# Pyrokine/LineSegmentDetector-SLAM

Measured on AMD Instinct MI355X. Metric: Mpixels/sec LSD (grad+grow+NFA), higher is better.
Workload: dtype f64; 1 GPU; 512 x 2048x2048 u8 occupancy maps per GPU tiled/rolled/flipped from 4 aisle-class fixtures (SURVEY 8d C4), full pipeline incl. lineIm, params 0.3/0.6/22.5/0.7/1024; images_total=512, images_rank0=512, parallelism=single GPU, rccl_gather_in_step=False, steps_in_flight=8, steps_in_flight_asked=8, region_waves_per_image=4, help_across_workgroups=False, last_steps_with_help=0, writeback_map=False

## Files before the change

### include/lsd_hip.h

```cpp
#ifndef LSD_HIP_H
#define LSD_HIP_H
#include <stddef.h>
#include <stdint.h>

#ifdef __cplusplus
extern "C" {
#endif

#define LSD_ABI_VERSION 1

enum {
    LSD_OK = 0,
    LSD_ERR_INVALID = 1,
    LSD_ERR_NO_DEVICE = 2,
    LSD_ERR_HIP = 3,
    LSD_ERR_UNSUPPORTED = 4,
    LSD_ERR_CAPACITY = 5,
    LSD_ERR_NOMEM = 6,
    LSD_ERR_INTERNAL = 7
};

typedef struct lsd_params {
    double sca;
    double sig;
// ... 236 lines not shown
                      const lsd_grid_match_rec *records, lsd_map_param map_param, double range_max, const uint8_t *corr,
                      double ang_step, lsd_grid_response_par response, lsd_grid_response_rec *out, uint32_t *volume);

void lsd_scaled_size(int cols, int rows, double sca, int *w, int *h);

enum { LSD_STAGE_ALL = 0, LSD_STAGE_GAUSS = 1, LSD_STAGE_GRAD = 2, LSD_STAGE_SORT = 3, LSD_STAGE_REGION = 4 };
int lsd_set_stop_after(lsd_ctx *ctx, int stage);
int lsd_set_trace(lsd_ctx *ctx, int on);
int lsd_set_fused_front(lsd_ctx *ctx, int on);
int lsd_set_region_waves(lsd_ctx *ctx, int waves);
int lsd_set_region_help(lsd_ctx *ctx, int waves);
int lsd_set_cost_history(lsd_ctx *ctx, int on);
int lsd_debug_set_stamp_budget(lsd_ctx *ctx, unsigned grows);
int lsd_debug_set_tuning(lsd_ctx *ctx, const char *name, int value);

enum { LSD_DBG_GAUSS = 1, LSD_DBG_MAG, LSD_DBG_DEG, LSD_DBG_STATE, LSD_DBG_ORDER, LSD_DBG_ORDER_VAL,
       LSD_DBG_NB, LSD_DBG_MAXGRAD, LSD_DBG_RECS, LSD_DBG_SEEDS, LSD_DBG_NSEED, LSD_DBG_STATS };
int lsd_debug_fetch(lsd_ctx *ctx, int image, int what, void *out, size_t bytes);

int lsd_debug_eval_math(lsd_ctx *ctx, int fn, const double *a, const double *b, double *out0, double *out1, size_t n);

int lsd_debug_lines(lsd_ctx *ctx, const double *recs, int n, int cols, int rows, lsd_line *lines_out, uint8_t *line_im);

int lsd_debug_calibrate(lsd_ctx *ctx, size_t bytes);

int lsd_last_timings(lsd_ctx *ctx, float ms_out[6]);

#ifdef __cplusplus
}
#endif
#endif
```

### linesegmentdetector-slam_amd/__init__.py

```python
import ctypes as C
import os

import numpy as np

_HERE = os.path.dirname(os.path.abspath(__file__))
LIB_PATH = os.path.join(_HERE, "liblsdhip.so")

LSD_OK, LSD_ERR_INVALID, LSD_ERR_NO_DEVICE, LSD_ERR_HIP, LSD_ERR_UNSUPPORTED, LSD_ERR_CAPACITY, LSD_ERR_NOMEM, LSD_ERR_INTERNAL = range(8)
LSD_FLAG_WRITEBACK_MAP = 1
STAGE_ALL, STAGE_GAUSS, STAGE_GRAD, STAGE_SORT, STAGE_REGION = range(5)
(DBG_GAUSS, DBG_MAG, DBG_DEG, DBG_STATE, DBG_ORDER, DBG_ORDER_VAL, DBG_NB, DBG_MAXGRAD, DBG_RECS, DBG_SEEDS,
 DBG_NSEED, DBG_STATS) = range(1, 13)

lsd_sca, lsd_sig, lsd_angThre, lsd_denThre, pseBin = 0.3, 0.6, 22.5, 0.7, 1024
z_occ_max_dis = 1.0
HOST_MAX_LINES_DEFAULT = 8192
rdp_leastPoint, rdp_threLine, rdp_leastDist = 3, 0.08, 0.5


class lsd_params(C.Structure):
    _fields_ = [("sca", C.c_double), ("sig", C.c_double), ("angThre", C.c_double), ("denThre", C.c_double),
                ("pseBin", C.c_int)]


# ... 162 lines not shown
    "lsd_enqueue_fa_carry_rebase_device": (_i, [_vp, _vp, _i, _vp, C.c_int32, lsd_map_frame, lsd_map_frame, _vp]),
    "lsd_enqueue_map_update_device": (_i, [_vp, _vp, _i, _i, _dbl, _dbl, _ppar, _vp, _vp, _vp, _i, _vp, _vp, _vp]),
    "lsd_reserve_map_update": (_i, [_vp, _i, _i]),
    "lsd_enqueue_scan_ingest_device": (_i, [_vp, _vp, _i, _i, _vp, _vp, _vp, _i, _vp]),
    "lsd_enqueue_laserscan_ingest_device": (_i, [_vp, _vp, _vp, _i, _i, _vp, _vp, _vp, _i, _vp]),
    "lsd_enqueue_grid_integrate_device": (_i, [_vp, _vp, _vp, _i, _i, _vp, _sz, lsd_map_param, _dbl, _vp, _vp, _vp]),
    "lsd_enqueue_grid_publish_device": (_i, [_vp, _vp, _vp, _sz, C.c_uint32, C.c_uint32, C.c_uint32, _vp, _vp]),
    "lsd_grid_integrate": (_i, [_vp, _vp, _vp, _i, _i, _vp, lsd_map_param, _dbl, _vp, _vp]),
    "lsd_enqueue_grid_likelihood_device": (_i, [_vp, _vp, _vp, _i, _i, C.c_uint32, C.c_uint32, C.c_uint32, lsd_grid_smear, _vp, _vp]),
    "lsd_grid_smear_default": (_i, [_dbl, _i, C.POINTER(lsd_grid_smear)]),
    "lsd_enqueue_grid_match_device": (_i, [_vp, _vp, _vp, _i, _i, _vp, _sz, lsd_map_param, _dbl, _vp, lsd_grid_search, _vp, _vp]),
    "lsd_grid_match": (_i, [_vp, _vp, _vp, _i, _i, _vp, lsd_map_param, _dbl, _vp, lsd_grid_search, _vp]),
    "lsd_grid_coarse_bytes": (_sz, [_i, _i, _i]),
    "lsd_enqueue_grid_coarse_device": (_i, [_vp, _vp, _i, _i, _i, _vp, _vp]),
    "lsd_enqueue_grid_match_mr_device": (_i, [_vp, _vp, _vp, _i, _i, _vp, _sz, lsd_map_param, _dbl, _vp, _vp, _i, lsd_grid_search, _vp, _vp, _vp]),
    "lsd_grid_match_mr": (_i, [_vp, _vp, _vp, _i, _i, _vp, lsd_map_param, _dbl, _vp, _i, lsd_grid_search, _vp, _vp]),
    "lsd_grid_response_volume_bytes": (_sz, [_i, lsd_grid_response]),
    "lsd_enqueue_grid_response_device": (_i, [_vp, _vp, _vp, _i, _i, _vp, _sz, _vp, lsd_map_param, _dbl, _vp, _dbl, lsd_grid_response, _vp, _vp,
                                              _vp]),
    "lsd_grid_response": (_i, [_vp, _vp, _vp, _i, _i, _vp, _vp, lsd_map_param, _dbl, _vp, _dbl, lsd_grid_response, _vp, _vp]),
    "lsd_debug_calibrate": (_i, [_vp, _sz]),
    "lsd_debug_eval_math": (_i, [_vp, _i, _vp, _vp, _vp, _vp, _sz]),
    "lsd_debug_lines": (_i, [_vp, _vp, _i, _i, _i, _vp, _vp]),
}
EXPORTED_SYMBOLS = list(_ABI)
del _vp, _i, _sz, _dbl, _pi, _ppar, _localize_args, _live_map_args, _maps_args

_lib = None


def load_library(path=None):
    global _lib
    if _lib is not None and path is None:
        return _lib
    p = path or os.environ.get("LSD_HIP_LIB") or LIB_PATH
    try:
        import torch
    except ImportError:
        pass
    if not os.path.exists(p):
        raise ImportError("liblsdhip.so is not built (%s); run `python -c 'import __graft_entry__ as g; g.build()'` "
                          "-- there is no CPU fallback" % p)
    L = C.CDLL(p)
    for name, (restype, argtypes) in _ABI.items():
        try:
            fn = getattr(L, name)
# ... 489 lines not shown
        if what == DBG_STATE:
            return get(what, np.uint32, npx).reshape(h, w)
        if what == DBG_NB:
            return int(get(what, np.int32, 1)[0])
        if what == DBG_NSEED:
            return int(get(what, np.int32, 1)[0])
        if what == DBG_MAXGRAD:
            return float(get(what, np.float64, 1)[0])
        if what == DBG_ORDER:
            return get(what, np.uint32, npx)[:self.fetch(image, DBG_NB, shape_wh)]
        if what == DBG_ORDER_VAL:
            return get(what, np.uint16, npx)[:self.fetch(image, DBG_NB, shape_wh)]
        if what == DBG_STATS:
            v = get(what, np.int64, 48)
            d = dict(zip(("grow_calls", "grown_px", "nfa_calls", "rrr_calls", "rrr_passes", "rrr_sentinel_drops",
                          "rrr_oob_reads", "cycles_refill", "cycles_total", "cycles_grow", "cycles_rect",
                          "cycles_nfa", "cycles_mark", "small_bails", "wait_noslot", "seeds", "exact_angle_evals",
                          "tile_fetches", "batches", "cycles_tiles", "spec_redos", "spec_discards", "cycles_wait", "small_steps",
                          "refill_rounds", "cycles_eval", "cycles_sums", "cycles_refine", "cycles_small", "cycles_select", "cycles_commit",
                          "wait_noseed", "requeued_ahead", "cycles_eval_at_cursor", "depth_end", "nfa_min_abs_enc", "nfa_min_gap_enc", "help_exports", "help_evals", "near_ties",
                          "wd_commit", "wd_next", "wd_nseeds", "wd_state", "wd_nbig", "wd_lock", "wd_pend", "wd_wave"),
                         [int(x) for x in v]))
            d["set_answers"], d["sets_founded"] = int(v[41]), int(v[42])
            d["cycles_nfa_count"], d["nfa_tail_iters"] = int(v[43]), int(v[44])
            d["nfa_bracket_misses"] = int(v[40])
            for k in ("nfa_min_abs", "nfa_min_gap"):
                enc = d.pop(k + "_enc")
                d[k] = float("inf") if enc == 0 else float(np.array([0x7ff0000000000000 - enc], np.uint64).view(np.float64)[0])
            return d
        if what == DBG_SEEDS:
            ns = self.fetch(image, DBG_NSEED, shape_wh)
            return get(what, SEED_DTYPE, ns)
        raise ValueError(what)

    def eval_math(self, fn, a, b=None):
        a = np.ascontiguousarray(a, np.float64)
        b = None if b is None else np.ascontiguousarray(b, np.float64)
        o0, o1 = np.zeros_like(a), np.zeros_like(a)
        self._chk(self.L.lsd_debug_eval_math(self.h, fn, a.ctypes.data, None if b is None else b.ctypes.data,
                                             o0.ctypes.data, o1.ctypes.data, a.size))
        return o0, o1

    def debug_lines(self, recs, rows, cols, want_lineim=True):
        r = np.ascontiguousarray(recs, np.float64).reshape(-1, 4)
        lines = np.zeros(len(r), LINE_DTYPE)
        im = np.zeros((rows, cols), np.uint8) if want_lineim else None
        self._chk(self.L.lsd_debug_lines(self.h, r.ctypes.data, len(r), cols, rows, lines.ctypes.data, im.ctypes.data if want_lineim else None))
        return lines, im

    def fetch_recs(self, image, count):
        a = np.zeros(max(count * 12, 1), np.float64)
        self._chk(self.L.lsd_debug_fetch(self.h, image, DBG_RECS, a.ctypes.data, a.nbytes))
        return a[:count * 12].reshape(count, 12)


class structLSD:

    def __init__(self, lineIm, linesInfo):
        self.lineIm = lineIm
        self.linesInfo = linesInfo
        self.len_linesInfo = len(linesInfo)


_default_ctx = None


def default_context():
    global _default_ctx
    if _default_ctx is None:
        _default_ctx = Context(0)
    return _default_ctx
# ... 1063 lines not shown
```

### linesegmentdetector-slam_amd/csrc/k_region.hip

```cpp
#include "lsd_internal.h"
#include "devmath.h"

#ifndef LSD_REGION_NW
#define LSD_REGION_NW 4
#endif
#if LSD_REGION_NW == 8
#define RVAR w8
#else
#define RVAR w4
#endif

namespace lsdhip {
namespace RVAR {
#include "region/config.h"
#include "region/stats.h"
#include "region/lds.h"
#include "region/wave.h"
#include "region/tiles.h"
#include "region/grow.h"
#include "region/rect.h"
#include "region/nfa.h"
#include "region/eval.h"

#ifdef LSD_REGION_STATS
// ... 921 lines not shown
            P[22] = (double)((long long)(precise ? n1 + 1 : 0) + 32768ll * n2 + 32768ll * 32768ll * m_off);
            P[23] = (double)epoch_snap;
            rg.aux[k & (RW - 1)] = (uint32_t)(wave * NS + slot);
        }
        wg_fence();
        if (lane == 0) st_st(&rg.state[k & (RW - 1)], R_STASH);
        adv = true;
    }

    asm volatile("s_waitcnt vmcnt(0)" ::: "memory");
    if (wave == 0 && lane == 0 && !pool) {
        b.counts[img] = lds_ld(&s_abort) ? -1 : s_lines;
        if (b.nseed) b.nseed[img] = s_ntrace;
    }
    if (b.stats && !pool) {
        unsigned long long* st = reinterpret_cast<unsigned long long*>(b.stats + img * kStatWords);
        if (lane == 0 && wave == 0 && !lds_ld(&s_abort)) { b.stats[img * kStatWords + 45] = (long long)(__builtin_amdgcn_s_getreg((3 << 11) | 20) & 15); b.stats[img * kStatWords + 46] = rt_begin; b.stats[img * kStatWords + 47] = (long long)__builtin_amdgcn_s_memrealtime(); }
        if (lane == 0 && wave == 0) {
            long long tot = (long long)__builtin_amdgcn_s_memtime() - t_begin;
            const long long rt = ((long long)__builtin_amdgcn_s_memrealtime() - rt_begin) * 24;
            if (tot <= 0 || tot > 4 * rt + 1000000) tot = rt > 0 ? rt : 1;
            g_stat[c.wave][sslot(ST_TOTAL)] = (unsigned long long)tot; g_stat[c.wave][sslot(ST_SEEDS)] = (unsigned long long)nseeds; DSTAT(ST_DEPTHEND, lds_ld(&s_depth));
        }
        if (lane < ST_COUNT && !lds_ld(&s_abort) && (sslot(lane) != 11 || lane == ST_NFASLOW || kStatSlots == ST_COUNT)) {
            if (lane == ST_MINNFA || lane == ST_MINGAP) atomicMax(&st[lane], g_stat[c.wave][sslot(lane)]);
            else atomicAdd(&st[lane], g_stat[c.wave][sslot(lane)]);
        }
        g_stat[c.wave][sslot(ST_XHELP)] = 0ull;
        g_stat[c.wave][sslot(ST_MINNFA)] = 0ull; g_stat[c.wave][sslot(ST_MINGAP)] = 0ull; g_stat[c.wave][sslot(ST_NFASLOW)] = 0ull; g_stat[c.wave][sslot(ST_TIES)] = 0ull;
    }
    if (!b.xq) return;
    if (wave == 0 && !pool) {
        agent_release();
        if (lane == 0) { st_l2(&xr[2], 1u); atomicAdd(&xhdr[1], 1u); }
    }
    bool early = !pool && ld_l2(&xhdr[0]) < (uint32_t)nimg;
    if (early) {
        if (b.tun_early <= 0) return;
        int ok = 0;
        if (lane == 0) {
            if (atomicAdd(&xhdr[3], 1u) >= (uint32_t)(b.tun_early * NW)) atomicSub(&xhdr[3], 1u);
            else ok = 1;
        }
        if (!__builtin_amdgcn_readfirstlane(ok)) return;
    }

    if (lane < NS) slot_k_l = -1;
    int hx = -1, hj = 0, hidle = 0, hscan = 0;
// ... 136 lines not shown
#undef LT

__global__ __launch_bounds__(64 * NW, LSD_REGION_WAVES_PER_SIMD) void k_region(Geom g, Buffers b, uint32_t id_base) {
#if LSD_REGION_NW == 8
    __shared__ int s_take;
    while (true) {
        int bid = (int)blockIdx.x, nimg = (int)gridDim.x - b.npool;
        if (b.pcount) {
            if (threadIdx.x == 0) s_take = atomicAdd(b.pcount, 1);
            __syncthreads();
            bid = s_take; nimg = b.nimg;
            __syncthreads();
            if (bid >= nimg) return;
        }
        region_image(g, b, id_base, bid, nimg);
        if (!b.pcount) return;
        __syncthreads();
    }
#else
    region_image(g, b, id_base, (int)blockIdx.x, (int)gridDim.x - b.npool);
#endif
}

}

#if LSD_REGION_NW == 8
void launch_region_w8(const Geom& g, const Buffers& b, int n, uint32_t id_base, hipStream_t s) {
    hipLaunchKernelGGL(w8::k_region, dim3(n + b.npool), dim3(64 * w8::NW), 0, s, g, b, id_base);
}
int region_slots() { return w8::NS; }
int region_waves() { return w8::NW; }
int region_ring() { return w8::RW; }
#else
void launch_region_w4(const Geom& g, const Buffers& b, int n, uint32_t id_base, hipStream_t s) {
    hipLaunchKernelGGL(w4::k_region, dim3(n + b.npool), dim3(64 * w4::NW), 0, s, g, b, id_base);
}
#endif

}
```

### linesegmentdetector-slam_amd/csrc/lsd_ctx.hip

```cpp
#include <math.h>
#include <stddef.h>
#include <stdio.h>
#include <stdlib.h>
#include <string.h>

#include <algorithm>
#include <mutex>
#include <string>
#include <vector>

#include "lsd_devbuf.h"
#include "lsd_internal.h"
#include "k1_lds.h"
#include "k_rdp_lds.h"

using namespace lsdhip;

struct Workspace {
    size_t cap_gpx = 0;
    size_t cap_n = 0, cap_npx = 0, cap_ws = 0;
    int cap_max_lines = 0;
    DevBuf<double> gauss, mag, deg, recs, recs_scaled;
    DevBuf<double2> sc;
    DevBuf<uint32_t> order;
// ... 1746 lines not shown
    HIPCHK(c, hipMemcpy(out0, d0.get(), n * 8, hipMemcpyDeviceToHost));
    HIPCHK(c, hipMemcpy(out1, d1.get(), n * 8, hipMemcpyDeviceToHost));
    return LSD_OK;
}

int lsd_debug_lines(lsd_ctx* c, const double* recs, int n, int cols, int rows, lsd_line* lines_out, uint8_t* line_im) {
    if (!c || !recs || !lines_out || n <= 0 || cols <= 0 || rows <= 0) return LSD_ERR_INVALID;
    HIPCHK(c, hipSetDevice(c->device));
    DevBuf<double> dr; DevBuf<int32_t> dn; DevBuf<lsd_line> dl; DevBuf<uint8_t> di;
    const size_t px = (size_t)cols * rows;
    HIPCHK(c, dr.resize((size_t)n * 4)); HIPCHK(c, dn.resize(1)); HIPCHK(c, dl.resize(n));
    if (line_im) HIPCHK(c, di.resize(px));
    HIPCHK(c, hipMemcpy(dr.get(), recs, (size_t)n * 4 * 8, hipMemcpyHostToDevice));
    HIPCHK(c, hipMemcpy(dn.get(), &n, 4, hipMemcpyHostToDevice));
    HIPCHK(c, hipMemsetAsync(dl.get(), 0xFF, (size_t)n * sizeof(lsd_line), c->stream));
    if (line_im) launch_clear(di.get(), px, c->num_cus, c->stream);
    launch_lines_of(dr.get(), dn.get(), dl.get(), line_im ? di.get() : nullptr, n, cols, rows, c->stream);
    HIPCHK(c, hipStreamSynchronize(c->stream));
    HIPCHK(c, hipMemcpy(lines_out, dl.get(), (size_t)n * sizeof(lsd_line), hipMemcpyDeviceToHost));
    if (line_im) HIPCHK(c, hipMemcpy(line_im, di.get(), px, hipMemcpyDeviceToHost));
    return LSD_OK;
}

}
```

### linesegmentdetector-slam_amd/csrc/lsd_internal.h

```cpp
#pragma once
#include <hip/hip_runtime.h>
#include <stdint.h>
#include "../../include/lsd_hip.h"

namespace lsdhip {

constexpr double kPi = 3.14159265358979323846;
constexpr int kCentreCount = 32768;
constexpr int kMaxTapRadius = 40;
constexpr int kLgTable = 16384;
constexpr int kLgTableMax = 1 << 23;
constexpr int kStatWords = 48;
constexpr int kStatTiesWord = 39;
constexpr int kStatTotalWord = 8;
constexpr int kPTable = 16;
constexpr int kXStride = 768, kXReq = 64, kXHdr = 16;

struct Geom {
    int W, H;
    int w, h;
    int npx;
    int gp;
    double sca;
    int tapR;
// ... 65 lines not shown
    int lg_count;
    const double* ptab;
    void* seeds;
    int32_t* nseed;
    long long* stats;
};

struct SeedRec {
    int order_idx, x, y, num, outcome, final_num;
    double logNFA;
};

hipError_t prepare_gauss(const Geom& g);
void launch_gauss(const Geom& g, const Buffers& b, int n, uint8_t* clr, bool remapped, hipStream_t s);
bool front_fits(const Geom& g, size_t max_lds);
void launch_front(const Geom& g, const Buffers& b, int n, uint8_t* clr, hipStream_t s);
void launch_remap_writeback(const Geom& g, const Buffers& b, int n, hipStream_t s);
void launch_gradient(const Geom& g, const Buffers& b, int n, hipStream_t s);
void launch_sort(const Geom& g, const Buffers& b, int n, hipStream_t s);
void launch_ordv(const double* mag, const unsigned long long* maxbits, const uint32_t* ord, uint16_t* out, int count, int pseBin, hipStream_t s);
void launch_order(const Buffers& b, int n, int npx, const long long* hist, hipStream_t s);
void launch_region_w4(const Geom& g, const Buffers& b, int n, uint32_t id_base, hipStream_t s);
void launch_region_w8(const Geom& g, const Buffers& b, int n, uint32_t id_base, hipStream_t s);
int region_slots();
int region_waves();
int region_ring();
void launch_calib(double* buf, size_t n, hipStream_t s);
void launch_match(const double* map_cache, int cols, int rows, const lsd_line* map_lines, const lsd_line* scan_lines,
                  const double* pts, int n_points, double lidx, double lidy, double lastx, double lasty, const int* pairs,
                  int n_pairs, double zmax, double max_esti_dist, double* out, hipStream_t s);
void launch_occ_to_map(const uint8_t* in, uint8_t* out, size_t n, hipStream_t s);
void launch_mapcache_spread(const uint8_t* maps, double* out, unsigned long long* claim, uint32_t* fr_a, uint32_t* fr_b, int* ctl,
                            int* cnt, int n, int G, int W, int H, double res, double zmax, int cell_radius, hipStream_t s);
void launch_mapcache(const uint8_t* maps, double* out, unsigned long long* claim, uint32_t* fr_a, uint32_t* fr_b, int n,
                     int W, int H, double res, double zmax, int cell_radius, hipStream_t s);
void launch_lines(const Geom& g, const Buffers& b, int n, hipStream_t s);
void launch_lines_of(const double* recs_scaled, const int32_t* count, lsd_line* lines, uint8_t* line_im, int n, int W, int H, hipStream_t s);
void launch_clear(uint8_t* p, size_t bytes, int num_cus, hipStream_t s);
void launch_compact_lines(const lsd_line* lines, const int32_t* counts, int max_lines, int n, lsd_line* flat, int32_t* offsets, hipStream_t s);
void launch_rdp(const double* scans, const int* lens, int n, int stride, int oriMapCol, int oriMapRow, double mapResol, double mapOriX,
                double mapOriY, int region_point_limit, double thre_line, double line_dist_thre_m, lsd_line* lines_out, int* n_lines,
                double* pts_out, int pts_cap, int* n_pts, double* lidar_pos, int* im_size, hipStream_t s);
void launch_rdp_maps(const double* scans, const int* lens, int n, int stride, const lsd_map_ref* maps, int n_maps, const int32_t* map_of,
                     int scans_per_seq, int region_point_limit, double thre_line, double line_dist_thre_m, lsd_line* lines_out, int* n_lines,
                     double* pts_out, int pts_cap, int* n_pts, double* lidar_pos, int* im_size, hipStream_t s);
int rdp_max_len();
// ... 62 lines not shown
```

### linesegmentdetector-slam_amd/csrc/region/nfa.h

```cpp
__device__ __forceinline__ double log_gamma_dev(const double* lgamma, int lg_count, int x) {
    if (x >= 0 && x < lg_count) return lgamma[x];
    const double xd = x;
    return 0.918938533204673 + (xd - 0.5) * log(xd) - xd +
           0.5 * xd * log(xd * sinh(1.0 / xd) + 1.0 / (810 * pow(xd, 6.0)));
}

template <int NP>
__device__ __forceinline__ int nfa_count(const RCtx& c, const Rec& rec, const double (&prec)[NP], int (&ali)[NP]) {
    const int lane = c.lane, xLim = c.w, yLim = c.h;
    STAT(ST_NFA, NP);
    [[maybe_unused]] const long long t00 = NOW();
    double verX[4], verY[4];
    verX[0] = rec.x1 - rec.dy * rec.wid / 2.0;
    verX[1] = rec.x2 - rec.dy * rec.wid / 2.0;
    verX[2] = rec.x2 + rec.dy * rec.wid / 2.0;
    verX[3] = rec.x1 + rec.dy * rec.wid / 2.0;
    verY[0] = rec.y1 + rec.dx * rec.wid / 2.0;
    verY[1] = rec.y2 + rec.dx * rec.wid / 2.0;
    verY[2] = rec.y2 - rec.dx * rec.wid / 2.0;
    verY[3] = rec.y1 - rec.dx * rec.wid / 2.0;
    int offset;
    if ((rec.x1 < rec.x2) && (rec.y1 <= rec.y2)) offset = 0;
    else if ((rec.x1 >= rec.x2) && (rec.y1 < rec.y2)) offset = 1;
    else if ((rec.x1 > rec.x2) && (rec.y1 >= rec.y2)) offset = 2;
    else offset = 3;
    const double vx0 = verX[offset & 3], vx1 = verX[(offset + 1) & 3], vx2 = verX[(offset + 2) & 3],
                 vx3 = verX[(offset + 3) & 3];
    const double vy0 = verY[offset & 3], vy1 = verY[(offset + 1) & 3], vy2 = verY[(offset + 2) & 3],
                 vy3 = verY[(offset + 3) & 3];
    const double cx0 = ceil(vx0);
    int xlen = cvt_x86(cx0 - floor(vx2));
    if (xlen < 0 && xlen != (int)0x80000000) xlen = -xlen;
    xlen = (int)((unsigned)xlen + 1u);
    const double k0 = (vy1 - vy0) / (vx1 - vx0);
    const double k1 = (vy2 - vy1) / (vx2 - vx1);
    const double k2 = (vy2 - vy3) / (vx2 - vx3);
    const double k3 = (vy3 - vy0) / (vx3 - vx0);
    int all = 0;
    #pragma unroll
    for (int q = 0; q < NP; q++) ali[q] = 0;
    const bool axis0 = axis_exact(rec.dx, rec.dy);
    const double ex_ = rec.x2 - rec.x1, ey_ = rec.y2 - rec.y1;
    const double cnz = kTieCoord * (fabs(rec.x1) + fabs(rec.y1) + fabs(ex_) + fabs(ey_) + rec.wid + 1.0);
    int ties_a = 0;
    int ties = (lane == 0 && !axis0 && (fabs(vx0 - rint(vx0)) <= cnz || fabs(vx2 - rint(vx2)) <= cnz)) ? 1 : 0;
    int* const s_incl = reinterpret_cast<int*>(G_WL(c.wave));
    int* const s_lo = s_incl + 64;
    int* const s_x = s_incl + 128;
    for (int cb = 0; cb < xlen; cb += 64) {
        const int i = cb + lane;
        int cntc = 0, lo = 0, xr = 0;
        if (i < xlen) {
            xr = cvt_x86(i + cx0);
            int yLow, yHigh;
            const double eLow = xr < vx3 ? vy0 + (xr - vx0) * k3 : vy3 + (xr - vx3) * k2;
            const double eHigh = xr < vx1 ? vy0 + (xr - vx0) * k0 : vy1 + (xr - vx1) * k1;
            yLow = cvt_x86(ceil(eLow));
            yHigh = cvt_x86(floor(eHigh));
            const double kLow = xr < vx3 ? k3 : k2, kHigh = xr < vx1 ? k0 : k1;
            if (!axis0 && (fabs(eLow - rint(eLow)) <= cnz * (1.0 + fabs(kLow)) || fabs(eHigh - rint(eHigh)) <= cnz * (1.0 + fabs(kHigh)) ||
                           fabs(xr - vx3) <= cnz || fabs(xr - vx1) <= cnz)) {
                ties++;
#ifdef LSD_TIE_PRINT
                printf("edge tie: xr %d eLow %.17g eHigh %.17g vx0 %.17g vx1 %.17g vx3 %.17g dx %.17g dy %.17g wid %.17g x1 %.17g y1 %.17g\n", xr, eLow, eHigh, vx0, vx1, vx3, rec.dx, rec.dy, rec.wid, rec.x1, rec.y1);
#endif
            }
            if (xr >= 0 && xr < xLim) {
                lo = yLow < 0 ? 0 : yLow;
                const int hi = yHigh > yLim - 1 ? yLim - 1 : yHigh;
                if (hi >= lo) cntc = hi - lo + 1;
            }
        }
        int inc = cntc;
        for (int off = 1; off < 64; off <<= 1) {
            const int t = __shfl_up(inc, off);
            if (lane >= off) inc += t;
        }
        const int tot = __builtin_amdgcn_readlane(inc, 63);
        if (tot == 0) continue;
        s_incl[lane] = inc; s_lo[lane] = lo; s_x[lane] = xr;
        all += tot;
        for (int t0 = 0; t0 < tot; t0 += 64) {
            const int t = t0 + lane;
            double df = 1e300;
            if (t < tot) {
                int ci = 0;
                for (int step = 32; step >= 1; step >>= 1)
                    if (s_incl[ci + step - 1] <= t) ci += step;
                const int ex = ci ? s_incl[ci - 1] : 0;
                const int j = s_lo[ci] + (t - ex);
                df = angle_diff(rec.deg, c.deg[(size_t)j * xLim + s_x[ci]]);
            }
            bool near = false;
            #pragma unroll
            for (int q = 0; q < NP; q++) {
                ali[q] += __builtin_popcountll(ballot64(df < prec[q]));
                near = near || fabs(df - prec[q]) <= 4.0 * kTieAng;
            }
            if (near) ties_a++;
        }
    }
    for (int off = 32; off >= 1; off >>= 1) { ties += __shfl_xor(ties, off); ties_a += __shfl_xor(ties_a, off); }
    TIES_AT(TS_EDGE, ties);
    TIES_AT(TS_ALIGN, ties_a);
    PSTAT(ST_NFACNT, NOW() - t00);
    return all;
}

struct NfaVal { double v; int flags; };
__device__ __noinline__ NfaVal nfa_tail(int all, int ali, int pk, double p, double logNT, const double* ptab, const double* lgamma, int lg_count) {
    if (all == 0 || ali == 0) return NfaVal{-logNT, 1};
    const double logp = ptab[pk * 3 + 0], log10p = ptab[pk * 3 + 1], log1mp = ptab[pk * 3 + 2];
    if (all == ali) return NfaVal{-logNT - all * log10p, 1};
    const double proTerm = p / (1.0 - p);
    const double log1Coef = log_gamma_dev(lgamma, lg_count, all + 1) - log_gamma_dev(lgamma, lg_count, ali + 1) - log_gamma_dev(lgamma, lg_count, all - ali + 1);
    const double log1Term = log1Coef + ali * logp + (all - ali) * log1mp;
    double term = exp_g(log1Term);
    const double eps = 2.2204e-16;
    if (fabs(term) < 100 * eps) {
        if (ali > all * p) return NfaVal{-log10_g(term) - logNT, 0};
        return NfaVal{-logNT, 1};
    }
    int nslow = 0;
    double binTail = term;
    const double tole = 0.1;
    constexpr double kOcmlBracket = 0x1p-44, kTiny = 0x1p-1000;
    for (int i = ali + 1; i <= all; i++) {
        const double binTerm = (all - i + 1) / (i * 1.0);
        const double multTerm = binTerm * proTerm;
        term *= multTerm;
        binTail += term;
        if (binTerm < 1) {
            const double N = (double)(all - i + 1), om = 1.0 - multTerm;
            const double Pd = pow(multTerm, N), Ld = log10(binTail);
            const double Pe = Pd * kOcmlBracket + kTiny, Le = fabs(Ld) * kOcmlBracket + kTiny;
            const double err_hi = term * ((1 - (Pd - Pe)) / om - 1), err_lo = term * ((1 - (Pd + Pe)) / om - 1);
            const double a1 = -(Ld - Le) - logNT, a2 = -(Ld + Le) - logNT;
            const double f1 = fabs(a1), f2 = fabs(a2);
            const double rhs_hi = tole * fmax(f1, f2) * binTail;
            const double rhs_lo = (a1 > 0) == (a2 > 0) && a1 != 0 && a2 != 0 ? tole * fmin(f1, f2) * binTail : 0.0;
            bool stop;
            if (err_hi < rhs_lo) stop = true;
            else if (!(err_lo < rhs_hi)) stop = false;
            else {
                nslow++;
                const double err = term * ((1 - pow_g(multTerm, N)) / om - 1);
                stop = err < tole * fabs(-log10_g(binTail) - logNT) * binTail;
            }
            if (stop) break;
        }
    }
    return NfaVal{-log10_g(binTail) - logNT, nslow << 8};
}

__device__ __noinline__ double improve(int cw_) {
    RCtx c = g_ctx[__builtin_amdgcn_readfirstlane(cw_)];
    c.lane = (int)(threadIdx.x & 63u);
    const int lane = c.lane;
    const double delt = 0.5, delt2 = delt / 2.0;
    Rec& best = g_ws[c.wave].rec;
    double bestNFA = 0;
    [[maybe_unused]] const long long t0 = NOW();
    auto margins = [&](double v, bool host_only, bool first) {
        if (fabs(v) <= 1.7976931348623157e308) {
            const double nv = 0x1p-51 * fabs(v + c.logNT) + 0x1p-52 * (1.0 + fmax(fabs(v), c.logNT));
            if (!host_only) STATMAX(ST_MINNFA, kInfBits - (unsigned long long)__double_as_longlong(fabs(v) / nv));
            int tie = (!host_only && fabs(v) / nv < 2.0) ? 1 : 0;
            if (!first && v != bestNFA) {
                const double nb = 0x1p-51 * fabs(bestNFA + c.logNT) + 0x1p-52 * (1.0 + fmax(fabs(bestNFA), c.logNT));
                STATMAX(ST_MINGAP, kInfBits - (unsigned long long)__double_as_longlong(fabs(v - bestNFA) / (nv + nb)));
                if (fabs(v - bestNFA) / (nv + nb) < 2.0) tie++;
            }
            TIES_AT(TS_NFA, tie);
        }
    };
    {
        Rec r = best;
        const double pr[1] = {r.prec};
        int al[1];
        const int all = nfa_count<1>(c, r, pr, al);
        const NfaVal nv = nfa_tail(all, al[0], r.pk, r.p, c.logNT, c.ptab, c.lgamma, c.lg_count);
        STAT(ST_NFASLOW, nv.flags >> 8);
        margins(nv.v, (nv.flags & 1) != 0, true);
        bestNFA = nv.v;
    }
    auto next_try = [&](Rec& r, int ph) -> bool {
        if (ph == 0 || ph == 4) { r.p /= 2.0; r.prec = r.p * kPi; r.pk++; return true; }
        if (!(r.wid - delt >= 0.5)) return false;
        if (ph == 2) { r.x1 -= r.dy * delt2; r.y1 += r.dx * delt2; r.x2 -= r.dy * delt2; r.y2 += r.dx * delt2; }
        else if (ph == 3) { r.x1 += r.dy * delt2; r.y1 -= r.dx * delt2; r.x2 += r.dy * delt2; r.y2 -= r.dx * delt2; }
        r.wid -= delt;
        return true;
    };
    for (int ph = 0; ph < 5 && !(bestNFA > 0); ph++) {
        int my_all = 0, my_ali = 0, my_pk = 0;
        double my_p = 0.0;
        bool my_eval = false;
        Rec r = best;
        if (ph == 0 || ph == 4) {
            double pr[5];
            int al[5];
            #pragma unroll
            for (int t = 0; t < 5; t++) pr[t] = r.p / (double)(2 << t) * kPi;
            const int all = nfa_count<5>(c, r, pr, al);
            #pragma unroll
            for (int t = 0; t < 5; t++)
                if (lane == t) { my_all = all; my_ali = al[t]; my_pk = r.pk + t + 1; my_p = r.p / (double)(2 << t); my_eval = true; }
        } else {
            for (int t = 0; t < 5; t++) {
                if (!next_try(r, ph)) continue;
                const double pr[1] = {r.prec};
                int al[1];
                const int all = nfa_count<1>(c, r, pr, al);
                if (lane == t) { my_all = all; my_ali = al[0]; my_pk = r.pk; my_p = r.p; my_eval = true; }
            }
        }
        NfaVal nv{0.0, 0};
        if (my_eval) nv = nfa_tail(my_all, my_ali, my_pk, my_p, c.logNT, c.ptab, c.lgamma, c.lg_count);
        r = best;
        for (int t = 0; t < 5; t++) {
            if (!next_try(r, ph)) continue;
            const double v = rl(nv.v, t);
            const int fl = __builtin_amdgcn_readlane(nv.flags, t);
            STAT(ST_NFASLOW, fl >> 8);
            margins(v, (fl & 1) != 0, false);
            if (v > bestNFA) { bestNFA = v; best = r; }
        }
    }
    PSTAT(ST_TNFA, NOW() - t0);
    return bestNFA;
}
```

### linesegmentdetector-slam_amd/csrc/region/stats.h

```cpp
enum { ST_GROW = 0, ST_GROWN, ST_NFA, ST_RRR, ST_RRRPASS, ST_SENT, ST_OOB, ST_TREFILL, ST_TOTAL, ST_TGROW, ST_TRECT, ST_TNFA,
       ST_TMARK, ST_SMALLBAIL, ST_WNOSLOT, ST_SEEDS, ST_EXACT, ST_WRING, ST_BATCHES, ST_TTILES, ST_REDO, ST_DISCARD,
       ST_WAIT, ST_SMALLSTEPS, ST_SLOW, ST_TEVAL, ST_TSUMS, ST_TREFINE, ST_TSMALL, ST_TSELECT, ST_TCOMMIT, ST_WNOSEED,
       ST_DEPTHUP, ST_DEPTHDN, ST_DEPTHEND, ST_MINNFA, ST_MINGAP, ST_XEXP, ST_XHELP, ST_TIES, ST_NFASLOW, ST_SETHIT, ST_SETNEW, ST_NFACNT, ST_NFAITER, ST_COUNT };
static_assert(ST_TOTAL == kStatTotalWord, "lsd_last_region_cycles reads this word");
static_assert(ST_TIES == kStatTiesWord, "lsd_last_sensitivity reads this word");
#ifdef LSD_REGION_STATS
constexpr int kStatSlots = ST_COUNT;
__device__ constexpr int sslot(int i) { return i; }
#else
constexpr int kStatSlots = 19;
__device__ constexpr int sslot(int i) {
    return i == ST_GROW ? 0 : i == ST_GROWN ? 1 : i == ST_NFA ? 2 : i == ST_RRR ? 3 : i == ST_RRRPASS ? 4 : i == ST_SENT ? 5 : i == ST_OOB ? 6 :
           i == ST_TOTAL ? 7 : i == ST_SEEDS ? 8 : i == ST_REDO ? 9 : i == ST_DISCARD ? 10 : i == ST_MINNFA ? 12 : i == ST_MINGAP ? 13 : i == ST_XEXP ? 14 : i == ST_XHELP ? 15 : i == ST_SETHIT ? 16 : i == ST_SETNEW ? 17 : i == ST_TIES ? 18 : 11;
}
#endif
#define STAT(i, v) do { g_stat[c.wave][sslot(i)] += (unsigned long long)(v); } while (0)
#define STATMAX(i, v) do { const unsigned long long n_ = (v); if (n_ > g_stat[c.wave][sslot(i)]) g_stat[c.wave][sslot(i)] = n_; } while (0)
constexpr unsigned long long kInfBits = 0x7ff0000000000000ull;
constexpr double kTieAng = 1e-15, kTieFlip = 1e-13, kTieRel = 1e-12, kTieCoord = 4e-15;
#ifdef LSD_TIE_SITES
__device__ constexpr unsigned long long tie_weight(int site) { unsigned long long w = 1; for (int i = 0; i < site; i++) w *= 1000ull; return w; }
#define TIE_UNIT(site) tie_weight(site)
#else
#define TIE_UNIT(site) 1ull
#endif
#define TIES_AT(site, v) STAT(ST_TIES, (unsigned long long)(v) * TIE_UNIT(site))
enum { TS_GROW = 0, TS_FLIP, TS_DENS, TS_DIST, TS_EDGE, TS_ALIGN, TS_NFA };
__device__ __forceinline__ bool axis_exact(double dx, double dy) { return fmin(fabs(dx), fabs(dy)) < 1e-15; }
#ifdef LSD_REGION_STATS
#define DSTAT(i, v) STAT(i, v)
#define NOW() ((long long)__builtin_amdgcn_s_memtime())
#else
#define DSTAT(i, v) do { } while (0)
#define NOW() 0ll
#endif
#ifdef LSD_REGION_BATCHPROF
#define BSTAT(i, v) DSTAT(i, v)
#define PSTAT(i, v) do { } while (0)
#else
#define BSTAT(i, v) do { } while (0)
#define PSTAT(i, v) DSTAT(i, v)
#endif
```

Baseline: 69120 Mpix/s.

## Count NFA pixels for all width/shift tries in one shared column sweep

For the width-reduction and shift phases of rectangle improvement, the change computes the pixel counts for all up to five candidate rectangles in one pass over the union of their columns. It records each try's row range in LDS and reads each gradient angle only once, instead of rescanning the image for every try. This is meant to cut repeated global loads and per-try scan overhead in improve(). In exchange it adds per-column recomputation of every try's rectangle geometry and a five-way membership test per pixel. It also adds a debug kernel that checks the counts and extra tail-timing stats, which only apply in stats builds.

New measurement: 68700 Mpix/s. No clear change (-0.6%).

```diff
diff --git a/include/lsd_hip.h b/include/lsd_hip.h
--- a/include/lsd_hip.h
+++ b/include/lsd_hip.h
@@ -282,6 +282,8 @@
 
 int lsd_debug_lines(lsd_ctx *ctx, const double *recs, int n, int cols, int rows, lsd_line *lines_out, uint8_t *line_im);
 
+int lsd_debug_nfa_counts(lsd_ctx *ctx, const double *deg, int cols, int rows, const double *recs, int n, int phase, int32_t *out);
+
 int lsd_debug_calibrate(lsd_ctx *ctx, size_t bytes);
 
 int lsd_last_timings(lsd_ctx *ctx, float ms_out[6]);
diff --git a/linesegmentdetector-slam_amd/__init__.py b/linesegmentdetector-slam_amd/__init__.py
--- a/linesegmentdetector-slam_amd/__init__.py
+++ b/linesegmentdetector-slam_amd/__init__.py
@@ -208,6 +208,7 @@
     "lsd_debug_calibrate": (_i, [_vp, _sz]),
     "lsd_debug_eval_math": (_i, [_vp, _i, _vp, _vp, _vp, _vp, _sz]),
     "lsd_debug_lines": (_i, [_vp, _vp, _i, _i, _i, _vp, _vp]),
+    "lsd_debug_nfa_counts": (_i, [_vp, _vp, _i, _i, _vp, _i, _i, _vp]),
 }
 EXPORTED_SYMBOLS = list(_ABI)
 del _vp, _i, _sz, _dbl, _pi, _ppar, _localize_args, _live_map_args, _maps_args
@@ -743,7 +744,8 @@
                           "wd_commit", "wd_next", "wd_nseeds", "wd_state", "wd_nbig", "wd_lock", "wd_pend", "wd_wave"),
                          [int(x) for x in v]))
             d["set_answers"], d["sets_founded"] = int(v[41]), int(v[42])
-            d["cycles_nfa_count"], d["nfa_tail_iters"] = int(v[43]), int(v[44])
+            d["cycles_nfa_count"] = int(v[43])
+            d["cycles_tail_exp"], d["cycles_tail_stop"], d["cycles_tail_log"] = (((int(v[44]) >> sh) & 0x1fffff) << 8 for sh in (0, 21, 42))
             d["nfa_bracket_misses"] = int(v[40])
             for k in ("nfa_min_abs", "nfa_min_gap"):
                 enc = d.pop(k + "_enc")
@@ -768,6 +770,15 @@
         im = np.zeros((rows, cols), np.uint8) if want_lineim else None
         self._chk(self.L.lsd_debug_lines(self.h, r.ctypes.data, len(r), cols, rows, lines.ctypes.data, im.ctypes.data if want_lineim else None))
         return lines, im
+
+    def debug_nfa_counts(self, deg, recs, phase):
+        if not hasattr(self.L, "lsd_debug_nfa_counts"):
+            raise LsdError(LSD_ERR_INVALID, "this liblsdhip.so predates lsd_debug_nfa_counts")
+        d = np.ascontiguousarray(deg, np.float64)
+        r = np.ascontiguousarray(recs, np.float64).reshape(-1, 12)
+        out = np.zeros((len(r), 2, 5, 2), np.int32)
+        self._chk(self.L.lsd_debug_nfa_counts(self.h, d.ctypes.data, d.shape[1], d.shape[0], r.ctypes.data, len(r), int(phase), out.ctypes.data))
+        return out
 
     def fetch_recs(self, image, count):
         a = np.zeros(max(count * 12, 1), np.float64)
diff --git a/linesegmentdetector-slam_amd/csrc/k_region.hip b/linesegmentdetector-slam_amd/csrc/k_region.hip
--- a/linesegmentdetector-slam_amd/csrc/k_region.hip
+++ b/linesegmentdetector-slam_amd/csrc/k_region.hip
@@ -967,8 +967,11 @@
             if (tot <= 0 || tot > 4 * rt + 1000000) tot = rt > 0 ? rt : 1;
             g_stat[c.wave][sslot(ST_TOTAL)] = (unsigned long long)tot; g_stat[c.wave][sslot(ST_SEEDS)] = (unsigned long long)nseeds; DSTAT(ST_DEPTHEND, lds_ld(&s_depth));
         }
-        if (lane < ST_COUNT && !lds_ld(&s_abort) && (sslot(lane) != 11 || lane == ST_NFASLOW || kStatSlots == ST_COUNT)) {
+        if (lane < ST_COUNT && !lds_ld(&s_abort) && (sslot(lane) != 11 || lane == ST_NFASLOW || kStatSlots >= ST_COUNT)) {
             if (lane == ST_MINNFA || lane == ST_MINGAP) atomicMax(&st[lane], g_stat[c.wave][sslot(lane)]);
+#ifdef LSD_REGION_STATS
+            else if (lane == ST_TAILPARTS) atomicAdd(&st[lane], tail_parts(g_stat[c.wave][ST_TTAILEXP], g_stat[c.wave][ST_TTAILSTOP], g_stat[c.wave][ST_TTAILLOG]));
+#endif
             else atomicAdd(&st[lane], g_stat[c.wave][sslot(lane)]);
         }
         g_stat[c.wave][sslot(ST_XHELP)] = 0ull;
@@ -1151,6 +1154,38 @@
 #endif
 }
 
+#if LSD_REGION_NW == 4
+__global__ __launch_bounds__(64) void k_nfa_counts(const double* deg, int w, int h, const double* recs, int n, int ph, int* out) {
+    RCtx c;
+    c.w = w; c.h = h; c.lane = (int)threadIdx.x; c.wave = 0; c.deg = deg;
+    const int lane = c.lane;
+    if (lane < kStatSlots) g_stat[0][lane] = 0ull;
+    for (int k = 0; k < n; k++) {
+        const double* f = recs + (size_t)k * 12;
+        Rec best;
+        best.x1 = f[0]; best.y1 = f[1]; best.x2 = f[2]; best.y2 = f[3]; best.wid = f[4]; best.cX = f[5]; best.cY = f[6]; best.deg = f[7];
+        best.dx = f[8]; best.dy = f[9]; best.p = f[10]; best.prec = f[11]; best.pk = 0;
+        int* const o = out + (size_t)k * 20;
+        Rec r = best;
+        int nt = 0;
+        for (int t = 0; t < 5; t++)
+            if (next_try(r, ph)) nt++;
+        int a = -1, b = -1;
+        if (nt >= 1 && !nfa_count_tries(c, best, ph, nt, a, b)) { a = -2; b = -2; }
+        if (lane < 5) { o[lane * 2] = lane < nt ? a : -1; o[lane * 2 + 1] = lane < nt ? b : -1; }
+        r = best;
+        for (int t = 0; t < 5; t++) {
+            int all = -1, al[1] = {-1};
+            if (next_try(r, ph)) {
+                const double pr[1] = {r.prec};
+                all = nfa_count<1>(c, r, pr, al);
+            }
+            if (lane == 0) { o[10 + t * 2] = all; o[10 + t * 2 + 1] = al[0]; }
+        }
+    }
+}
+#endif
+
 }
 
 #if LSD_REGION_NW == 8
@@ -1164,6 +1199,9 @@
 void launch_region_w4(const Geom& g, const Buffers& b, int n, uint32_t id_base, hipStream_t s) {
     hipLaunchKernelGGL(w4::k_region, dim3(n + b.npool), dim3(64 * w4::NW), 0, s, g, b, id_base);
 }
+void launch_nfa_counts(const double* deg, int w, int h, const double* recs, int n, int ph, int* out, hipStream_t s) {
+    hipLaunchKernelGGL(w4::k_nfa_counts, dim3(1), dim3(64), 0, s, deg, w, h, recs, n, ph, out);
+}
 #endif
 
 }
diff --git a/linesegmentdetector-slam_amd/csrc/lsd_ctx.hip b/linesegmentdetector-slam_amd/csrc/lsd_ctx.hip
--- a/linesegmentdetector-slam_amd/csrc/lsd_ctx.hip
+++ b/linesegmentdetector-slam_amd/csrc/lsd_ctx.hip
@@ -1792,4 +1792,23 @@
     return LSD_OK;
 }
 
-}
+int lsd_debug_nfa_counts(lsd_ctx* c, const double* deg, int cols, int rows, const double* recs, int n, int phase, int32_t* out) {
+    if (!c || !deg || !recs || !out || n <= 0 || cols <= 0 || rows <= 0 || cols >= 32766 || rows >= 32766 || phase < 1 || phase > 3) return LSD_ERR_INVALID;
+    for (int k = 0; k < n; k++) {
+        const double* f = recs + (size_t)k * 12;
+        for (int j = 0; j < 12; j++)
+            if (!(fabs(f[j]) <= (j == 8 || j == 9 ? 1.0000001 : 65536.0))) return LSD_ERR_INVALID;
+    }
+    HIPCHK(c, hipSetDevice(c->device));
+    DevBuf<double> dd, dr; DevBuf<int32_t> dout;
+    const size_t px = (size_t)cols * rows;
+    HIPCHK(c, dd.resize(px)); HIPCHK(c, dr.resize((size_t)n * 12)); HIPCHK(c, dout.resize((size_t)n * 20));
+    HIPCHK(c, hipMemcpy(dd.get(), deg, px * 8, hipMemcpyHostToDevice));
+    HIPCHK(c, hipMemcpy(dr.get(), recs, (size_t)n * 12 * 8, hipMemcpyHostToDevice));
+    launch_nfa_counts(dd.get(), cols, rows, dr.get(), n, phase, dout.get(), c->stream);
+    HIPCHK(c, hipStreamSynchronize(c->stream));
+    HIPCHK(c, hipMemcpy(out, dout.get(), (size_t)n * 20 * 4, hipMemcpyDeviceToHost));
+    return LSD_OK;
+}
+
+}
diff --git a/linesegmentdetector-slam_amd/csrc/lsd_internal.h b/linesegmentdetector-slam_amd/csrc/lsd_internal.h
--- a/linesegmentdetector-slam_amd/csrc/lsd_internal.h
+++ b/linesegmentdetector-slam_amd/csrc/lsd_internal.h
@@ -111,6 +111,7 @@
 void launch_order(const Buffers& b, int n, int npx, const long long* hist, hipStream_t s);
 void launch_region_w4(const Geom& g, const Buffers& b, int n, uint32_t id_base, hipStream_t s);
 void launch_region_w8(const Geom& g, const Buffers& b, int n, uint32_t id_base, hipStream_t s);
+void launch_nfa_counts(const double* deg, int w, int h, const double* recs, int n, int ph, int* out, hipStream_t s);
 int region_slots();
 int region_waves();
 int region_ring();
diff --git a/linesegmentdetector-slam_amd/csrc/region/nfa.h b/linesegmentdetector-slam_amd/csrc/region/nfa.h
--- a/linesegmentdetector-slam_amd/csrc/region/nfa.h
+++ b/linesegmentdetector-slam_amd/csrc/region/nfa.h
@@ -5,11 +5,13 @@
            0.5 * xd * log(xd * sinh(1.0 / xd) + 1.0 / (810 * pow(xd, 6.0)));
 }
 
-template <int NP>
-__device__ __forceinline__ int nfa_count(const RCtx& c, const Rec& rec, const double (&prec)[NP], int (&ali)[NP]) {
-    const int lane = c.lane, xLim = c.w, yLim = c.h;
-    STAT(ST_NFA, NP);
-    [[maybe_unused]] const long long t00 = NOW();
+struct RectScan {
+    double vx0, vx1, vx2, vx3, vy0, vy1, vy2, vy3, k0, k1, k2, k3, cx0, cnz;
+    int xlen;
+    bool axis0;
+};
+__device__ __forceinline__ RectScan rect_scan(const Rec& rec) {
+    RectScan s;
     double verX[4], verY[4];
     verX[0] = rec.x1 - rec.dy * rec.wid / 2.0;
     verX[1] = rec.x2 - rec.dy * rec.wid / 2.0;
@@ -24,26 +26,59 @@
     else if ((rec.x1 >= rec.x2) && (rec.y1 < rec.y2)) offset = 1;
     else if ((rec.x1 > rec.x2) && (rec.y1 >= rec.y2)) offset = 2;
     else offset = 3;
-    const double vx0 = verX[offset & 3], vx1 = verX[(offset + 1) & 3], vx2 = verX[(offset + 2) & 3],
-                 vx3 = verX[(offset + 3) & 3];
-    const double vy0 = verY[offset & 3], vy1 = verY[(offset + 1) & 3], vy2 = verY[(offset + 2) & 3],
-                 vy3 = verY[(offset + 3) & 3];
-    const double cx0 = ceil(vx0);
-    int xlen = cvt_x86(cx0 - floor(vx2));
+    s.vx0 = verX[offset & 3]; s.vx1 = verX[(offset + 1) & 3]; s.vx2 = verX[(offset + 2) & 3]; s.vx3 = verX[(offset + 3) & 3];
+    s.vy0 = verY[offset & 3]; s.vy1 = verY[(offset + 1) & 3]; s.vy2 = verY[(offset + 2) & 3]; s.vy3 = verY[(offset + 3) & 3];
+    s.cx0 = ceil(s.vx0);
+    int xlen = cvt_x86(s.cx0 - floor(s.vx2));
     if (xlen < 0 && xlen != (int)0x80000000) xlen = -xlen;
-    xlen = (int)((unsigned)xlen + 1u);
-    const double k0 = (vy1 - vy0) / (vx1 - vx0);
-    const double k1 = (vy2 - vy1) / (vx2 - vx1);
-    const double k2 = (vy2 - vy3) / (vx2 - vx3);
-    const double k3 = (vy3 - vy0) / (vx3 - vx0);
+    s.xlen = (int)((unsigned)xlen + 1u);
+    s.k0 = (s.vy1 - s.vy0) / (s.vx1 - s.vx0);
+    s.k1 = (s.vy2 - s.vy1) / (s.vx2 - s.vx1);
+    s.k2 = (s.vy2 - s.vy3) / (s.vx2 - s.vx3);
+    s.k3 = (s.vy3 - s.vy0) / (s.vx3 - s.vx0);
+    s.axis0 = axis_exact(rec.dx, rec.dy);
+    const double ex_ = rec.x2 - rec.x1, ey_ = rec.y2 - rec.y1;
+    s.cnz = kTieCoord * (fabs(rec.x1) + fabs(rec.y1) + fabs(ex_) + fabs(ey_) + rec.wid + 1.0);
+    return s;
+}
+__device__ __forceinline__ bool corner_tie(const RectScan& s) {
+    return !s.axis0 && (fabs(s.vx0 - rint(s.vx0)) <= s.cnz || fabs(s.vx2 - rint(s.vx2)) <= s.cnz);
+}
+__device__ __forceinline__ int col_rows(const RectScan& s, int xr, int xLim, int yLim, int& lo, int& ties) {
+    const double eLow = xr < s.vx3 ? s.vy0 + (xr - s.vx0) * s.k3 : s.vy3 + (xr - s.vx3) * s.k2;
+    const double eHigh = xr < s.vx1 ? s.vy0 + (xr - s.vx0) * s.k0 : s.vy1 + (xr - s.vx1) * s.k1;
+    const int yLow = cvt_x86(ceil(eLow));
+    const int yHigh = cvt_x86(floor(eHigh));
+    const double kLow = xr < s.vx3 ? s.k3 : s.k2, kHigh = xr < s.vx1 ? s.k0 : s.k1;
+    if (!s.axis0 && (fabs(eLow - rint(eLow)) <= s.cnz * (1.0 + fabs(kLow)) || fabs(eHigh - rint(eHigh)) <= s.cnz * (1.0 + fabs(kHigh)) ||
+                     fabs(xr - s.vx3) <= s.cnz || fabs(xr - s.vx1) <= s.cnz)) {
+        ties++;
+#ifdef LSD_TIE_PRINT
+        printf("edge tie: xr %d eLow %.17g eHigh %.17g vx0 %.17g vx1 %.17g vx3 %.17g\n", xr, eLow, eHigh, s.vx0, s.vx1, s.vx3);
+#endif
+    }
+    int cntc = 0;
+    lo = 0;
+    if (xr >= 0 && xr < xLim) {
+        lo = yLow < 0 ? 0 : yLow;
+        const int hi = yHigh > yLim - 1 ? yLim - 1 : yHigh;
+        if (hi >= lo) cntc = hi - lo + 1;
+    }
+    return cntc;
+}
+
+template <int NP>
+__device__ __forceinline__ int nfa_count(const RCtx& c, const Rec& rec, const double (&prec)[NP], int (&ali)[NP]) {
+    const int lane = c.lane, xLim = c.w, yLim = c.h;
+    STAT(ST_NFA, NP);
+    [[maybe_unused]] const long long t00 = NOW();
+    const RectScan s = rect_scan(rec);
+    const int xlen = s.xlen;
     int all = 0;
     #pragma unroll
     for (int q = 0; q < NP; q++) ali[q] = 0;
-    const bool axis0 = axis_exact(rec.dx, rec.dy);
-    const double ex_ = rec.x2 - rec.x1, ey_ = rec.y2 - rec.y1;
-    const double cnz = kTieCoord * (fabs(rec.x1) + fabs(rec.y1) + fabs(ex_) + fabs(ey_) + rec.wid + 1.0);
     int ties_a = 0;
-    int ties = (lane == 0 && !axis0 && (fabs(vx0 - rint(vx0)) <= cnz || fabs(vx2 - rint(vx2)) <= cnz)) ? 1 : 0;
+    int ties = (lane == 0 && corner_tie(s)) ? 1 : 0;
     int* const s_incl = reinterpret_cast<int*>(G_WL(c.wave));
     int* const s_lo = s_incl + 64;
     int* const s_x = s_incl + 128;
@@ -51,25 +86,8 @@
         const int i = cb + lane;
         int cntc = 0, lo = 0, xr = 0;
         if (i < xlen) {
-            xr = cvt_x86(i + cx0);
-            int yLow, yHigh;
-            const double eLow = xr < vx3 ? vy0 + (xr - vx0) * k3 : vy3 + (xr - vx3) * k2;
-            const double eHigh = xr < vx1 ? vy0 + (xr - vx0) * k0 : vy1 + (xr - vx1) * k1;
-            yLow = cvt_x86(ceil(eLow));
-            yHigh = cvt_x86(floor(eHigh));
-            const double kLow = xr < vx3 ? k3 : k2, kHigh = xr < vx1 ? k0 : k1;
-            if (!axis0 && (fabs(eLow - rint(eLow)) <= cnz * (1.0 + fabs(kLow)) || fabs(eHigh - rint(eHigh)) <= cnz * (1.0 + fabs(kHigh)) ||
-                           fabs(xr - vx3) <= cnz || fabs(xr - vx1) <= cnz)) {
-                ties++;
-#ifdef LSD_TIE_PRINT
-                printf("edge tie: xr %d eLow %.17g eHigh %.17g vx0 %.17g vx1 %.17g vx3 %.17g dx %.17g dy %.17g wid %.17g x1 %.17g y1 %.17g\n", xr, eLow, eHigh, vx0, vx1, vx3, rec.dx, rec.dy, rec.wid, rec.x1, rec.y1);
-#endif
-            }
-            if (xr >= 0 && xr < xLim) {
-                lo = yLow < 0 ? 0 : yLow;
-                const int hi = yHigh > yLim - 1 ? yLim - 1 : yHigh;
-                if (hi >= lo) cntc = hi - lo + 1;
-            }
+            xr = cvt_x86(i + s.cx0);
+            cntc = col_rows(s, xr, xLim, yLim, lo, ties);
         }
         int inc = cntc;
         for (int off = 1; off < 64; off <<= 1) {
@@ -107,15 +125,113 @@
     return all;
 }
 
+__device__ __forceinline__ bool next_try(Rec& r, int ph) {
+    const double delt = 0.5, delt2 = delt / 2.0;
+    if (ph == 0 || ph == 4) { r.p /= 2.0; r.prec = r.p * kPi; r.pk++; return true; }
+    if (!(r.wid - delt >= 0.5)) return false;
+    if (ph == 2) { r.x1 -= r.dy * delt2; r.y1 += r.dx * delt2; r.x2 -= r.dy * delt2; r.y2 += r.dx * delt2; }
+    else if (ph == 3) { r.x1 += r.dy * delt2; r.y1 -= r.dx * delt2; r.x2 += r.dy * delt2; r.y2 -= r.dx * delt2; }
+    r.wid -= delt;
+    return true;
+}
+
+constexpr int kNoRows = 0x7fff;
+static_assert(WLW >= 7 * 64, "nfa_count_tries keeps 7 x 64 ints in the worklist's place");
+__device__ __forceinline__ bool nfa_count_tries(const RCtx& c, const Rec& best, int ph, int nt, int& my_all, int& my_ali) {
+    const int lane = c.lane, xLim = c.w, yLim = c.h;
+    [[maybe_unused]] const long long t00 = NOW();
+    int* const s_incl = reinterpret_cast<int*>(G_WL(c.wave));
+    int* const s_lo = s_incl + 64;
+    int* const s_pair = s_incl + 128;
+    int X0 = 0x7fffffff, X1 = -0x7fffffff;
+    int ties = 0, ties_a = 0;
+    bool sane = true;
+    {
+        Rec r = best;
+        #pragma unroll 1
+        for (int t = 0; t < nt; t++) {
+            (void)next_try(r, ph);
+            const RectScan s = rect_scan(r);
+            sane = sane && fabs(s.cx0) <= 1048576.0 && s.xlen >= 1 && s.xlen <= 1048576;
+            const int xa = cvt_x86(s.cx0);
+            X0 = min(X0, xa); X1 = max(X1, xa + s.xlen);
+            if (lane == 0 && corner_tie(s)) ties++;
+        }
+    }
+    if (!sane) return false;
+    STAT(ST_NFA, nt);
+    my_all = 0; my_ali = 0;
+    const double prec = best.prec;
+    #pragma unroll
+    for (int q = 0; q < 5; q++) s_pair[q * 64 + lane] = kNoRows;
+    for (int xb = X0; xb < X1; xb += 64) {
+        const int xr = xb + lane;
+        int ulo = 0x7fffffff, uhi = -1;
+        Rec r = best;
+        #pragma unroll 1
+        for (int t = 0; t < nt; t++) {
+            (void)next_try(r, ph);
+            const RectScan s = rect_scan(r);
+            const int i = xr - cvt_x86(s.cx0);
+            int lo = 0, cntc = 0;
+            if (i >= 0 && i < s.xlen) cntc = col_rows(s, xr, xLim, yLim, lo, ties);
+            const int hi = lo + cntc - 1;
+            s_pair[t * 64 + lane] = cntc ? (lo | (hi << 16)) : kNoRows;
+            if (cntc) { ulo = min(ulo, lo); uhi = max(uhi, hi); }
+            int tot = cntc;
+            for (int off = 32; off >= 1; off >>= 1) tot += __shfl_xor(tot, off);
+            if (lane == t) my_all += tot;
+        }
+        int inc = uhi >= ulo ? uhi - ulo + 1 : 0;
+        for (int off = 1; off < 64; off <<= 1) {
+            const int t = __shfl_up(inc, off);
+            if (lane >= off) inc += t;
+        }
+        const int tot = __builtin_amdgcn_readlane(inc, 63);
+        if (tot == 0) continue;
+        s_incl[lane] = inc; s_lo[lane] = ulo;
+        for (int t0 = 0; t0 < tot; t0 += 64) {
+            const int t = t0 + lane;
+            double df = 1e300;
+            int ci = 0, j = -1;
+            if (t < tot) {
+                for (int step = 32; step >= 1; step >>= 1)
+                    if (s_incl[ci + step - 1] <= t) ci += step;
+                const int ex = ci ? s_incl[ci - 1] : 0;
+                j = s_lo[ci] + (t - ex);
+                df = angle_diff(best.deg, c.deg[(size_t)j * xLim + (xb + ci)]);
+            }
+            const bool ok = df < prec;
+            int nin = 0;
+            #pragma unroll
+            for (int q = 0; q < 5; q++) {
+                const int pr = s_pair[q * 64 + ci];
+                const bool in = j >= (pr & 0xffff) && j <= (pr >> 16);
+                const int n = __builtin_popcountll(ballot64(in && ok));
+                if (lane == q) my_ali += n;
+                nin += in ? 1 : 0;
+            }
+            if (fabs(df - prec) <= 4.0 * kTieAng) ties_a += nin;
+        }
+    }
+    for (int off = 32; off >= 1; off >>= 1) { ties += __shfl_xor(ties, off); ties_a += __shfl_xor(ties_a, off); }
+    TIES_AT(TS_EDGE, ties);
+    TIES_AT(TS_ALIGN, ties_a);
+    PSTAT(ST_NFACNT, NOW() - t00);
+    return true;
+}
+
 struct NfaVal { double v; int flags; };
 __device__ __noinline__ NfaVal nfa_tail(int all, int ali, int pk, double p, double logNT, const double* ptab, const double* lgamma, int lg_count) {
     if (all == 0 || ali == 0) return NfaVal{-logNT, 1};
     const double logp = ptab[pk * 3 + 0], log10p = ptab[pk * 3 + 1], log1mp = ptab[pk * 3 + 2];
     if (all == ali) return NfaVal{-logNT - all * log10p, 1};
+    [[maybe_unused]] const long long ta = NOW();
     const double proTerm = p / (1.0 - p);
     const double log1Coef = log_gamma_dev(lgamma, lg_count, all + 1) - log_gamma_dev(lgamma, lg_count, ali + 1) - log_gamma_dev(lgamma, lg_count, all - ali + 1);
     const double log1Term = log1Coef + ali * logp + (all - ali) * log1mp;
     double term = exp_g(log1Term);
+    LSTAT(ST_TTAILEXP, NOW() - ta);
     const double eps = 2.2204e-16;
     if (fabs(term) < 100 * eps) {
         if (ali > all * p) return NfaVal{-log10_g(term) - logNT, 0};
@@ -131,6 +247,7 @@
         term *= multTerm;
         binTail += term;
         if (binTerm < 1) {
+            [[maybe_unused]] const long long ts = NOW();
             const double N = (double)(all - i + 1), om = 1.0 - multTerm;
             const double Pd = pow(multTerm, N), Ld = log10(binTail);
             const double Pe = Pd * kOcmlBracket + kTiny, Le = fabs(Ld) * kOcmlBracket + kTiny;
@@ -147,17 +264,20 @@
                 const double err = term * ((1 - pow_g(multTerm, N)) / om - 1);
                 stop = err < tole * fabs(-log10_g(binTail) - logNT) * binTail;
             }
+            LSTAT(ST_TTAILSTOP, NOW() - ts);
             if (stop) break;
         }
     }
-    return NfaVal{-log10_g(binTail) - logNT, nslow << 8};
+    [[maybe_unused]] const long long tl = NOW();
+    const double logTail = log10_g(binTail);
+    LSTAT(ST_TTAILLOG, NOW() - tl);
+    return NfaVal{-logTail - logNT, nslow << 8};
 }
 
 __device__ __noinline__ double improve(int cw_) {
     RCtx c = g_ctx[__builtin_amdgcn_readfirstlane(cw_)];
     c.lane = (int)(threadIdx.x & 63u);
     const int lane = c.lane;
-    const double delt = 0.5, delt2 = delt / 2.0;
     Rec& best = g_ws[c.wave].rec;
     double bestNFA = 0;
     [[maybe_unused]] const long long t0 = NOW();
@@ -184,14 +304,6 @@
         margins(nv.v, (nv.flags & 1) != 0, true);
         bestNFA = nv.v;
     }
-    auto next_try = [&](Rec& r, int ph) -> bool {
-        if (ph == 0 || ph == 4) { r.p /= 2.0; r.prec = r.p * kPi; r.pk++; return true; }
-        if (!(r.wid - delt >= 0.5)) return false;
-        if (ph == 2) { r.x1 -= r.dy * delt2; r.y1 += r.dx * delt2; r.x2 -= r.dy * delt2; r.y2 += r.dx * delt2; }
-        else if (ph == 3) { r.x1 += r.dy * delt2; r.y1 -= r.dx * delt2; r.x2 += r.dy * delt2; r.y2 -= r.dx * delt2; }
-        r.wid -= delt;
-        return true;
-    };
     for (int ph = 0; ph < 5 && !(bestNFA > 0); ph++) {
         int my_all = 0, my_ali = 0, my_pk = 0;
         double my_p = 0.0;
@@ -207,12 +319,20 @@
             for (int t = 0; t < 5; t++)
                 if (lane == t) { my_all = all; my_ali = al[t]; my_pk = r.pk + t + 1; my_p = r.p / (double)(2 << t); my_eval = true; }
         } else {
-            for (int t = 0; t < 5; t++) {
-                if (!next_try(r, ph)) continue;
-                const double pr[1] = {r.prec};
-                int al[1];
-                const int all = nfa_count<1>(c, r, pr, al);
-                if (lane == t) { my_all = all; my_ali = al[0]; my_pk = r.pk; my_p = r.p; my_eval = true; }
+            int nt = 0;
+            for (int t = 0; t < 5; t++)
+                if (next_try(r, ph)) nt++;
+            r = best;
+            if (nt >= 2 && nfa_count_tries(c, r, ph, nt, my_all, my_ali)) {
+                if (lane < nt) { my_pk = r.pk; my_p = r.p; my_eval = true; }
+            } else {
+                for (int t = 0; t < 5; t++) {
+                    if (!next_try(r, ph)) continue;
+                    const double pr[1] = {r.prec};
+                    int al[1];
+                    const int all = nfa_count<1>(c, r, pr, al);
+                    if (lane == t) { my_all = all; my_ali = al[0]; my_pk = r.pk; my_p = r.p; my_eval = true; }
+                }
             }
         }
         NfaVal nv{0.0, 0};
diff --git a/linesegmentdetector-slam_amd/csrc/region/stats.h b/linesegmentdetector-slam_amd/csrc/region/stats.h
--- a/linesegmentdetector-slam_amd/csrc/region/stats.h
+++ b/linesegmentdetector-slam_amd/csrc/region/stats.h
@@ -1,11 +1,16 @@
 enum { ST_GROW = 0, ST_GROWN, ST_NFA, ST_RRR, ST_RRRPASS, ST_SENT, ST_OOB, ST_TREFILL, ST_TOTAL, ST_TGROW, ST_TRECT, ST_TNFA,
        ST_TMARK, ST_SMALLBAIL, ST_WNOSLOT, ST_SEEDS, ST_EXACT, ST_WRING, ST_BATCHES, ST_TTILES, ST_REDO, ST_DISCARD,
        ST_WAIT, ST_SMALLSTEPS, ST_SLOW, ST_TEVAL, ST_TSUMS, ST_TREFINE, ST_TSMALL, ST_TSELECT, ST_TCOMMIT, ST_WNOSEED,
-       ST_DEPTHUP, ST_DEPTHDN, ST_DEPTHEND, ST_MINNFA, ST_MINGAP, ST_XEXP, ST_XHELP, ST_TIES, ST_NFASLOW, ST_SETHIT, ST_SETNEW, ST_NFACNT, ST_NFAITER, ST_COUNT };
+       ST_DEPTHUP, ST_DEPTHDN, ST_DEPTHEND, ST_MINNFA, ST_MINGAP, ST_XEXP, ST_XHELP, ST_TIES, ST_NFASLOW, ST_SETHIT, ST_SETNEW, ST_NFACNT, ST_TAILPARTS, ST_COUNT,
+       ST_TTAILEXP = ST_COUNT, ST_TTAILSTOP, ST_TTAILLOG, ST_LDS_COUNT };
+static_assert(ST_COUNT <= 45, "words 45..47 of an image's counter record are the developer record of when and where the image ran");
+__device__ __forceinline__ unsigned long long tail_parts(unsigned long long e, unsigned long long s, unsigned long long l) {
+    return (e >> 8) | ((s >> 8) << 21) | ((l >> 8) << 42);
+}
 static_assert(ST_TOTAL == kStatTotalWord, "lsd_last_region_cycles reads this word");
 static_assert(ST_TIES == kStatTiesWord, "lsd_last_sensitivity reads this word");
 #ifdef LSD_REGION_STATS
-constexpr int kStatSlots = ST_COUNT;
+constexpr int kStatSlots = ST_LDS_COUNT;
 __device__ constexpr int sslot(int i) { return i; }
 #else
 constexpr int kStatSlots = 19;
@@ -30,9 +35,11 @@
 #ifdef LSD_REGION_STATS
 #define DSTAT(i, v) STAT(i, v)
 #define NOW() ((long long)__builtin_amdgcn_s_memtime())
+#define LSTAT(i, v) do { g_stat[threadIdx.x >> 6][sslot(i)] += (unsigned long long)(v); } while (0)
 #else
 #define DSTAT(i, v) do { } while (0)
 #define NOW() 0ll
+#define LSTAT(i, v) do { } while (0)
 #endif
 #ifdef LSD_REGION_BATCHPROF
 #define BSTAT(i, v) DSTAT(i, v)
```
